# xytpai/kfunca

Measured on AMD Instinct MI355X. Metric: bf16 GEMM TFLOP/s + causal-attn fwd+bwd tokens/s, higher is better.
Workload: dtype bf16

## Files before the change

### kfunca_amd/csrc/device/attention.hip

```cpp
#include <math.h>
#include <stdlib.h>

#include <algorithm>
#include <type_traits>

#include "common.h"

namespace kf {

typedef __attribute__((ext_vector_type(8))) __bf16 bf16x8;
typedef __attribute__((ext_vector_type(8))) _Float16 f16x8;
typedef __attribute__((ext_vector_type(4))) short s16x4;
typedef __attribute__((ext_vector_type(8))) short s16x8;
typedef __attribute__((ext_vector_type(16))) float f32x16;
typedef __attribute__((ext_vector_type(4))) float f32x4;

struct AttnArgs {
    const char *q, *k, *v, *o, *d_o;
    char *out, *dq, *dk, *dv;
    float *lse;
    const float *lse_r;
    float *delta;
    float *nlse, *ndelta;
    int64_t B, H, Sq, Skv, D;
// ... 735 lines not shown
    char *slab = smem + DQ_RING * FTILE + wid * DQ_RING * DQ_SLAB;
    int vo[DB][2];
#pragma unroll
    for (int d = 0; d < DB; ++d) {
        vo[d][0] = a_tr_lane_off(d * 32, 0);
        vo[d][1] = a_tr_lane_off(d * 32, 1);
    }
    const int grp = lane >> 4, qq = (lane >> 2) & 3, pp = lane & 3, h = grp >> 1;
    const unsigned smem_u = (unsigned)(uintptr_t)(const __attribute__((address_space(3))) char *)smem;
    const int sp = grp & 1;
    const unsigned ds_rd = smem_u + (unsigned)(slab - smem) + sp * 1024 + 64 * ((2 * h + (qq >> 1)) ^ (2 * sp)) + 32 * (qq & 1) + 16 * (pp & 1) + 8 * (pp >> 1);
    int ds_src[2];
#pragma unroll
    for (int pc = 0; pc < 2; ++pc) ds_src[pc] = pc * 1024 + (((lane >> 2) ^ (2 * pc)) * 4 + (lane & 3)) * 16;
    const int krow = lane >> 4, kpos = lane & 15;
#pragma nounroll
  for (int pass = 0; pass < (a.persist ? 2 * a.persist : 1); ++pass) {
    const int xp = xb0 + (pass >> 1) * nwx;
    const int xb = ((pass & 1) != (a.persist_rev != 0)) ? nxb - 1 - xp : xp;
    const int qblk = nxb - 1 - xb;
    const int64_t q0 = (int64_t)qblk * FQ, qw = q0 + wid * 32;
    const bool active = qw < a.Sq;
    const int sl = (int)(qw >> 5);
    f32x16 dq[DB];
#pragma unroll
    for (int d = 0; d < DB; ++d)
#pragma unroll
        for (int e = 0; e < 16; ++e) dq[d][e] = 0.f;
    const int64_t q_end = q0 + FQ < a.Sq ? q0 + FQ : a.Sq;
    const int64_t kv_end = a.Skv < q_end ? a.Skv : q_end;
    const int nt = (int)((kv_end + ABK - 1) / ABK);
    const char *dsg = a.ds + ((bh - a.bh0) * a.ds_pair + ds_row_base(qblk, a.ds_nkb, a.ds_tri) + wid) * DS_TILE;
    const int kwb_last = (int)(a.ds_nkb * 8 - 1);
    const int slw = qblk * 8 + wid;
    auto stage = [&](int tile, int slot) {
        const int tl = tile < nt ? tile : nt - 1;
        const int kfirst = tl * ABK, klast = (int)a.Skv - 1 - kfirst;
        const char *kg = Kg + (int64_t)kfirst * a.lk.sr;
#pragma unroll
        for (int i = 0; i < 2; ++i) {
            const int row0 = (wid * 2 + i) * 4, row = row0 + krow;
            const int chunk = kpos ^ (((row & 3) << 2) | ((row >> 2) & 3));
            const int srow = row < klast ? row : klast;
            if (D == AD || chunk < D / 8)
                __builtin_amdgcn_global_load_lds((const __attribute__((address_space(1))) void *)(kg + (int64_t)srow * a.lk.sr + chunk * 16),
                                                 (__attribute__((address_space(3))) void *)(smem + slot * FTILE + row0 * AROW), 16, 0, 0);
        }
#pragma unroll
        for (int hf = 0; hf < 2; ++hf) {
            int kwb = 2 * tl + hf;
            kwb = kwb < kwb_last ? kwb : kwb_last;
            kwb = kwb <= slw ? kwb : (slw < kwb_last ? slw : kwb_last);
            const char *tg = dsg + (int64_t)kwb * 8 * DS_TILE;
#pragma unroll
            for (int pc = 0; pc < 2; ++pc)
                __builtin_amdgcn_global_load_lds((const __attribute__((address_space(1))) void *)(tg + ds_src[pc]),
                                                 (__attribute__((address_space(3))) void *)(slab + slot * DQ_SLAB + hf * DS_TILE + pc * 1024), 16, 0, 0);
        }
    };
    stage(0, 0);
    stage(1, 1);
    for (int t = 0; t < nt; ++t) {
        asm volatile("s_waitcnt vmcnt(6)" ::: "memory");
        __builtin_amdgcn_s_barrier();
        asm volatile("" ::: "memory");
        stage(t + 2, (t + 2) % DQ_RING);
        const char *kt = smem + (t % DQ_RING) * FTILE;
        const unsigned dsb = ds_rd + (unsigned)((t % DQ_RING) * DQ_SLAB);
        if (active && 2 * t <= sl && !KF_MUT(3, t == 0 && qblk == nxb - 1)) {
            dq_step<BF, 0, 0, DB>(kt, vo, dsb, dq);
            dq_step<BF, 0, 1, DB>(kt, vo, dsb, dq);
            if (2 * t + 1 <= sl) {
                dq_step<BF, 1, 0, DB>(kt, vo, dsb, dq);
                dq_step<BF, 1, 1, DB>(kt, vo, dsb, dq);
            }
        }
    }
    asm volatile("s_waitcnt vmcnt(0)" ::: "memory");
    __syncthreads();
    if (active) a_store_rows<BF, DB>(smem + wid * 32 * OPAD, a.dq + a_head(a.ldq, bh, a.H) + qw * a.ldq.sr, dq, a.scale, a.ldq.sr,
                                     (int)(a.Sq - qw < 32 ? a.Sq - qw : 32));
    if (a.persist) __syncthreads();
  }
}

constexpr int BQS = 32;

constexpr int K4B = 128;
constexpr int K4SL = 2 * BQS * AROW + 256;
constexpr int K4PAIR = 2 * K4SL;
constexpr int K4LDS = 4 * K4PAIR;
constexpr bool K4_SPREAD = true;
static_assert(K4LDS >= 4 * 32 * OPAD, "epilogue slabs must fit");

template <int OFF>
__device__ __forceinline__ void k4_rows4(unsigned e, unsigned o, s16x8 (&f)[4]) {
    asm volatile("ds_read_b128 %0, %4 offset:%c6\n\tds_read_b128 %1, %5 offset:%c6\n\t"
                 "ds_read_b128 %2, %4 offset:%c7\n\tds_read_b128 %3, %5 offset:%c7"
                 : "=&v"(f[0]), "=&v"(f[1]), "=&v"(f[2]), "=&v"(f[3])
                 : "v"(e), "v"(o), "n"(OFF), "n"(OFF + 512)
                 : "memory");
}
template <int OFF>
__device__ __forceinline__ void k4_rowc(unsigned lr, f32x4 (&c)[4]) {
    asm volatile("ds_read_b128 %0, %4 offset:%c5\n\tds_read_b128 %1, %4 offset:%c6\n\t"
                 "ds_read_b128 %2, %4 offset:%c7\n\tds_read_b128 %3, %4 offset:%c8"
                 : "=&a"(c[0]), "=&a"(c[1]), "=&a"(c[2]), "=&a"(c[3])
                 : "v"(lr), "n"(OFF), "n"(OFF + 32), "n"(OFF + 64), "n"(OFF + 96)
                 : "memory");
}
struct K4Tr { s16x4 lo[4], hi[4]; };
template <int OFF>
__device__ __forceinline__ void k4_tr4(unsigned t0, unsigned t1, K4Tr &t) {
    asm volatile("ds_read_b64_tr_b16 %0, %8 offset:%c10\n\tds_read_b64_tr_b16 %1, %9 offset:%c10\n\t"
                 "ds_read_b64_tr_b16 %2, %8 offset:%c11\n\tds_read_b64_tr_b16 %3, %9 offset:%c11\n\t"
                 "ds_read_b64_tr_b16 %4, %8 offset:%c12\n\tds_read_b64_tr_b16 %5, %9 offset:%c12\n\t"
                 "ds_read_b64_tr_b16 %6, %8 offset:%c13\n\tds_read_b64_tr_b16 %7, %9 offset:%c13"
                 : "=&v"(t.lo[0]), "=&v"(t.hi[0]), "=&v"(t.lo[1]), "=&v"(t.hi[1]), "=&v"(t.lo[2]), "=&v"(t.hi[2]), "=&v"(t.lo[3]), "=&v"(t.hi[3])
                 : "v"(t0), "v"(t1), "n"(OFF), "n"(OFF + 512), "n"(OFF + 1024), "n"(OFF + 1536)
                 : "memory");
}
template <int N>
__device__ __forceinline__ void k4_wait4(s16x8 (&f)[4]) {
    asm volatile("s_waitcnt lgkmcnt(%c4)" : "+v"(f[0]), "+v"(f[1]), "+v"(f[2]), "+v"(f[3]) : "n"(N) : "memory");
}
template <int N>
__device__ __forceinline__ void k4_wait4c(s16x8 (&f)[4], f32x4 (&c)[4]) {
    asm volatile("s_waitcnt lgkmcnt(%c8)"
                 : "+v"(f[0]), "+v"(f[1]), "+v"(f[2]), "+v"(f[3]), "+a"(c[0]), "+a"(c[1]), "+a"(c[2]), "+a"(c[3])
                 : "n"(N)
                 : "memory");
}
template <int N>
__device__ __forceinline__ void k4_wait_tr(K4Tr &a) {
    asm volatile("s_waitcnt lgkmcnt(%c8)"
                 : "+v"(a.lo[0]), "+v"(a.hi[0]), "+v"(a.lo[1]), "+v"(a.hi[1]), "+v"(a.lo[2]), "+v"(a.hi[2]), "+v"(a.lo[3]), "+v"(a.hi[3])
                 : "n"(N)
                 : "memory");
}
template <bool BF>
__device__ __forceinline__ typename AFrag<BF>::type k4_frag(const K4Tr &t, int d) {
    s16x8 r;
    r[0] = t.lo[d][0]; r[1] = t.lo[d][1]; r[2] = t.lo[d][2]; r[3] = t.lo[d][3];
    r[4] = t.hi[d][0]; r[5] = t.hi[d][1]; r[6] = t.hi[d][2]; r[7] = t.hi[d][3];
    return __builtin_bit_cast(typename AFrag<BF>::type, r);
}
__device__ __forceinline__ f32x16 k4_acc(const f32x4 (&c)[4]) {
    f32x16 r;
#pragma unroll
    for (int g = 0; g < 4; ++g)
#pragma unroll
        for (int j = 0; j < 4; ++j) r[4 * g + j] = c[g][j];
    return r;
}

template <int OFF>
__device__ __forceinline__ void k4_rows4a(unsigned e, unsigned o, s16x8 (&f)[4]) {
    asm volatile("ds_read_b128 %0, %4 offset:%c6\n\tds_read_b128 %1, %5 offset:%c6\n\t"
                 "ds_read_b128 %2, %4 offset:%c7\n\tds_read_b128 %3, %5 offset:%c7"
                 : "=&a"(f[0]), "=&a"(f[1]), "=&a"(f[2]), "=&a"(f[3])
                 : "v"(e), "v"(o), "n"(OFF), "n"(OFF + 512)
                 : "memory");
}
template <int OFF>
__device__ __forceinline__ void k4_rowcv(unsigned lr, f32x4 (&c)[4]) {
    asm volatile("ds_read_b128 %0, %4 offset:%c5\n\tds_read_b128 %1, %4 offset:%c6\n\t"
// ... 1408 lines not shown
        return with_flags([&](auto BF, auto SQ) { return launch(attn_fwd_w4_kernel<BF, SQ>, grid, 256, KF_FWD_W4_LDS_BYTES, st, a); }, bf, sq);
    }
    KF_REQUIRE(!lays, KF_ERR_UNSUPPORTED, "kf_attn_fwd_strided: this shape / stride combination has no matrix-core kernel (ragged lengths want K and V with one row stride)");
    if (f32_mfma) {
        const size_t ldsx = std::max((size_t)2 * XK * (D + 4), (size_t)4 * 32 * (D + 4)) * sizeof(float);
        const int64_t nxx = (Sq + XQ - 1) / XQ;
        a.persist = pair_flag(nxx);
        KF_PROF("attn_fwd_f32_mfma", st);
        return launch(D == 128 ? attn_fwd_f32_mfma_kernel<128> : attn_fwd_f32_mfma_kernel<64>, (unsigned)((a.persist ? nxx / 2 : nxx) * B * H), 256, ldsx, st, a);
    }
    const int DP = (int)D + 1;
    const size_t lds = sizeof(float) * ((size_t)GQ * DP + (size_t)GK * DP + (size_t)GK * D + (size_t)GQ * (GK + 1) + GQ);
    KF_PROF("attn_fwd_generic", st);
    return launch(dtype == KF_F32 ? attn_fwd_generic_kernel<float> : bf ? attn_fwd_generic_kernel<bf16_t> : attn_fwd_generic_kernel<f16_t>,
                  dim3((unsigned)((Sq + GQ - 1) / GQ), (unsigned)(B * H)), 256, lds, st, a);
}

extern "C" int kf_attn_fwd(int dtype, int64_t B, int64_t H, int64_t Sq, int64_t Skv, int64_t D, const void *q,
                           const void *k, const void *v, void *o, float *lse, void *stream) {
    return kf_attn_fwd_scaled(dtype, B, H, Sq, Skv, D, D > 0 ? 1.0f / sqrtf((float)D) : 1.0f, q, k, v, o, lse, stream);
}

extern "C" int kf_attn_fwd_scaled(int dtype, int64_t B, int64_t H, int64_t Sq, int64_t Skv, int64_t D, float scale, const void *q,
                                  const void *k, const void *v, void *o, float *lse, void *stream) {
    return attn_fwd_impl(dtype, B, H, H, Sq, Skv, D, scale, q, k, v, o, lse, nullptr, stream);
}

static int attn_fwd_strided_impl(int dtype, int64_t B, int64_t H, int64_t Hkv, int64_t Sq, int64_t Skv, int64_t D, float scale, const void *q,
                                 const kf_attn_layout *lq, const void *k, const kf_attn_layout *lk, const void *v, const kf_attn_layout *lv,
                                 void *o, const kf_attn_layout *lo, float *lse, void *stream) {
    KF_REQUIRE(mfma16_ok(dtype, Sq, Skv, D), KF_ERR_UNSUPPORTED,
               "kf_attn_fwd_strided: strided layouts are served by the 16-bit matrix-core kernels only (D = 64 or 128; Skv >= Sq, or Sq, Skv multiples of 128)");
    AttnArgs::Lay lays[4];
    KF_REQUIRE(lay_from(lq, 2, lays[0]) && lay_from(lk, 2, lays[1]) && lay_from(lv, 2, lays[2]) && lay_from(lo, 2, lays[3]), KF_ERR_INVALID,
               "kf_attn_fwd_strided: strides must be non-negative multiples of 8 elements");
    KF_REQUIRE(((uintptr_t)q | (uintptr_t)k | (uintptr_t)v | (uintptr_t)o) % 16 == 0, KF_ERR_INVALID, "kf_attn_fwd_strided: operands must be 16-byte aligned");
    return attn_fwd_impl(dtype, B, H, Hkv, Sq, Skv, D, scale, q, k, v, o, lse, lays, stream);
}

extern "C" int kf_attn_fwd_strided(int dtype, int64_t B, int64_t H, int64_t Sq, int64_t Skv, int64_t D, float scale, const void *q,
                                   const kf_attn_layout *lq, const void *k, const kf_attn_layout *lk, const void *v, const kf_attn_layout *lv,
                                   void *o, const kf_attn_layout *lo, float *lse, void *stream) {
    return attn_fwd_strided_impl(dtype, B, H, H, Sq, Skv, D, scale, q, lq, k, lk, v, lv, o, lo, lse, stream);
}

extern "C" int kf_attn_bwd_workspace_bytes(int dtype, int64_t B, int64_t H, int64_t Sq, int64_t Skv, int64_t D,
                                           size_t *bytes) {
    KF_REQUIRE(bytes, KF_ERR_INVALID, "kf_attn_bwd_workspace_bytes: null out pointer");
    int rc = check_common("kf_attn_bwd_workspace_bytes", dtype, B, H, Sq, Skv, D);
    if (rc != KF_OK) return rc;
    *bytes = bwd_stats_bytes(B * H, Sq);
    if (mfma16_ok(dtype, Sq, Skv, D) && B * H > 0) {
        const DsPlan ds = ds_plan(B * H, Sq, Skv, ds_cap());
        *bytes += ds_bytes(ds.group, Sq, Skv, ds.tri);
    }
    return KF_OK;
}

static size_t gqa_part_bytes(int dtype, int64_t B, int64_t H, int64_t Hkv, int64_t Skv, int64_t D) {
    return H == Hkv ? 0 : a_align((size_t)B * H * Skv * D * (dtype == KF_F32 ? 4 : 2));
}

static int attn_dkv_group_sum(int dtype, int64_t B, int64_t Hkv, int64_t Skv, int64_t D, int G, const char *pk, const char *pv, void *dk, void *dv,
                              AttnArgs::Lay ldk, AttnArgs::Lay ldv, hipStream_t st) {
    constexpr int R = 4;
    const int es = dtype == KF_F32 ? 4 : 2, vec = 16 / es;
    const bool wide = D % vec == 0 && (((uintptr_t)dk | (uintptr_t)dv) % 16 == 0) &&
                      ((ldk.sb | ldk.sh | ldk.sr | ldv.sb | ldv.sh | ldv.sr) % 16 == 0);
    const int nparts = (int)(wide ? D / vec : D);
    int lg = 0;
    while ((1 << lg) < nparts && lg < 6) ++lg;
    const int64_t nrows = B * Hkv * Skv, rows_per_block = (int64_t)(256 >> lg) * R;
    const unsigned grid = (unsigned)((nrows + rows_per_block - 1) / rows_per_block);
    KF_PROF("attn_bwd_dkv_group_sum", st);
    auto go = [&](auto t) {
        using T = decltype(t);
        return wide ? launch(attn_dkv_group_sum_kernel<T, 16 / sizeof(T), R>, grid, 256, 0, st, pk, pv, (char *)dk, (char *)dv, ldk, ldv, nrows, Skv, Hkv, G,
                             nparts, lg)
                    : launch(attn_dkv_group_sum_kernel<T, 1, R>, grid, 256, 0, st, pk, pv, (char *)dk, (char *)dv, ldk, ldv, nrows, Skv, Hkv, G, nparts, lg);
    };
    return dtype == KF_F32 ? go(float{}) : dtype == KF_BF16 ? go(bf16_t{}) : go(f16_t{});
}

static int attn_bwd_kernels(int dtype, int64_t B, int64_t H, int64_t Hkv, int64_t Sq, int64_t Skv, int64_t D, float scale, const void *q, const void *k,
                            const void *v, const void *o, const float *lse, const void *d_o, void *dq, void *dk, void *dv, const AttnArgs::Lay *lays,
                            void *workspace, size_t workspace_bytes, void *stream) {
    int rc = check_common("kf_attn_bwd", dtype, B, H, Sq, Skv, D);
    if (rc != KF_OK) return rc;
    if (B * H == 0 || Sq == 0 || Skv == 0) return KF_OK;
    KF_REQUIRE(q && k && v && o && lse && d_o && dq && dk && dv, KF_ERR_INVALID, "kf_attn_bwd: null operand");
    const size_t stats = bwd_stats_bytes(B * H, Sq), part = gqa_part_bytes(dtype, B, H, Hkv, Skv, D);
    const size_t need = stats + 2 * part;
    KF_REQUIRE(workspace && workspace_bytes >= need, KF_ERR_WORKSPACE, "kf_attn_bwd: workspace of at least %zu bytes required, got %zu", need, workspace_bytes);
    AttnArgs a;
    if ((rc = attn_args(a, B, H, Hkv, Sq, Skv, D, scale, lays, 8)) != KF_OK) return rc;
    a.q = (const char *)q; a.k = (const char *)k; a.v = (const char *)v; a.o = (const char *)o; a.d_o = (const char *)d_o;
    a.dq = (char *)dq; a.dk = (char *)dk; a.dv = (char *)dv;
    if (part) {
        a.dk = (char *)workspace + stats;
        a.dv = a.dk + part;
        a.ldk = a.ldv = lay_contig(H, Skv, D, 2);
    }
    a.lse_r = lse; a.delta = (float *)workspace;
    a.Sqc = stat_rows(Sq);
    a.nlse = (float *)((char *)workspace + a_align((size_t)B * H * Sq * sizeof(float)));
    a.ndelta = (float *)((char *)a.nlse + a_align((size_t)B * H * a.Sqc * sizeof(float)));
    hipStream_t st = as_stream(stream);
    const int64_t nbh = B * H, nrows = nbh * Sq;
    const bool bf = dtype == KF_BF16, d64 = D == 64;
    const bool tiled = mfma_ok(dtype, Sq, Skv, D);
    const bool dkv_w4 = ((tiled && Skv % K5B == 0) || w4_any_ok(dtype, Sq, Skv, D)) && a.lk.sr == a.lv.sr && a.ldk.sr == a.ldv.sr &&
                        (uint64_t)(Sq + 32) * (uint64_t)std::max(a.lq.sr, a.ldo.sr) < (1ull << 32) && (uint64_t)K5B * (uint64_t)std::max(a.lk.sr, a.ldk.sr) < (1ull << 31) &&
                        (uint64_t)((const char *)a.ndelta - (const char *)a.nlse) < (1ull << 31) && !knob(KNOB_ATTN_DKV_V4);
    const DsPlan ds = ds_plan(nbh, Sq, Skv, workspace_bytes - need);
    const bool keep_ds = ds.group > 0;
    const bool mfma16 = tiled || (dkv_w4 && keep_ds);
    const bool f32_mfma = dtype == KF_F32 && (D == 64 || D == 128) && Sq % 32 == 0 && Skv % 32 == 0;
    if (mfma16) {
        const bool dkv_sq = dkv_w4 && D == AD && knob(KNOB_ATTN_SCALED_OPERANDS);
        const float rscale = dkv_sq ? kLog2e : 1.0f / scale;
        {
            KF_PROF("attn_bwd_delta", st);
            const int64_t nrows_c = nbh * a.Sqc;
            rc = launch(bf ? attn_delta_kernel<true, 2> : attn_delta_kernel<false, 2>, (unsigned)((nrows_c + 31) / 32), 256, 0, st, a.o, a.d_o, a.delta,
                        nrows_c, a.lse_r, a.nlse, a.ndelta, rscale, a.lo, a.ldo, Sq, H, (int)(D / 8), a.Sqc);
            if (rc != KF_OK) return rc;
        }
        a.ds = keep_ds ? (char *)workspace + need : nullptr;
        a.ds_tri = ds.tri;
        a.ds_pair = ds_pair_tiles(Sq, Skv, ds.tri);
        a.ds_nkb = (Skv + 255) / 256;
        const int64_t nkb4 = Skv / K4B, nkb5 = (Skv + K5B - 1) / K5B, nxq = (Sq + FQ - 1) / FQ;
        const int64_t grp = keep_ds ? ds.group : nbh;
        for (int64_t bh0 = 0; bh0 < nbh; bh0 += grp) {
            a.bh0 = bh0;
            a.nbh = (int)std::min<int64_t>(grp, nbh - bh0);
            a.xcd_map = (a.nbh % 8 == 0) && !knob(KNOB_ATTN_NO_XCD);
            {
                a.persist_rev = 1;
                KF_PROF(d64 ? "attn_bwd_dkv_mfma_d64" : "attn_bwd_dkv_mfma", st);
                if (dkv_w4) {
                    a.persist = pair_flag(nkb5);
                    const dim3 grid((unsigned)((a.persist ? nkb5 / 2 : nkb5) * a.nbh));
                    a.nvwg = grid.x;
                    if (d64)
                        rc = with_flags([&](auto BF, auto DS) { return launch(attn_bwd_dkv_w4_kernel<BF, DS, false, true>, grid, 256, KF_DKV_W4_LDS_BYTES, st, a); },
                                        bf, keep_ds);
                    else
                        rc = with_flags([&](auto BF, auto DS, auto SQ) { return launch(attn_bwd_dkv_w4_kernel<BF, DS, SQ>, grid, 256, KF_DKV_W4_LDS_BYTES, st, a); },
                                        bf, keep_ds, dkv_sq);
                } else {
                    a.persist = pair_flag(nkb4);
                    const dim3 grid((unsigned)((a.persist ? nkb4 / 2 : nkb4) * a.nbh));
                    rc = with_flags([&](auto BF, auto DS, auto D64) { return launch(attn_bwd_dkv_v4_kernel<BF, DS, D64 ? 64 : 128>, grid, 256, K4LDS, st, a); },
                                    bf, keep_ds, d64);
                }
                if (rc != KF_OK) return rc;
            }
            a.persist = pair_flag(nxq);
            a.persist_rev = 0;
            const dim3 grid((unsigned)((a.persist ? nxq / 2 : nxq) * a.nbh));
            if (keep_ds) {
                KF_PROF(d64 ? "attn_bwd_dq_mfma_d64" : "attn_bwd_dq_mfma", st);
                rc = with_flags([&](auto BF, auto D64) { return launch(attn_bwd_dq_ds_kernel<BF, D64 ? 64 : 128>, grid, FNT, DQ_LDS, st, a); }, bf, d64);
            } else {
                KF_PROF(d64 ? "attn_bwd_dq_mfma_split_d64" : "attn_bwd_dq_mfma_split", st);
                rc = with_flags([&](auto BF, auto D64) { return launch(attn_bwd_dq_v2_kernel<BF, D64 ? 64 : 128>, grid, FNT, QLDS, st, a); }, bf, d64);
            }
            if (rc != KF_OK) return rc;
        }
        return KF_OK;
    }
    KF_REQUIRE(!lays, KF_ERR_UNSUPPORTED, "kf_attn_bwd_strided: this shape / stride / workspace combination has no matrix-core kernel (ragged lengths want room for dS)");
    const unsigned gd = (unsigned)((nrows + 3) / 4);
    if (f32_mfma) {
        {
            KF_PROF("attn_bwd_delta", st);
            rc = launch(attn_delta_generic_kernel<float>, gd, 256, 0, st, (const float *)o, (const float *)d_o, a.delta, nrows, (int)D);
            if (rc != KF_OK) return rc;
        }
        const size_t tiles = (size_t)2 * XK * (D + 4) * sizeof(float) + 256, slabs = (size_t)4 * 32 * (D + 4) * sizeof(float);
        const size_t ldsx = std::max(tiles, slabs);
        const int64_t nxq = (Sq + XQ - 1) / XQ, nkb = (Skv + XQ - 1) / XQ;
        {
            a.persist = pair_flag(nkb);
            KF_PROF("attn_bwd_dkv_f32_mfma", st);
            rc = launch(D == 128 ? attn_bwd_dkv_f32_mfma_kernel<128> : attn_bwd_dkv_f32_mfma_kernel<64>, (unsigned)((a.persist ? nkb / 2 : nkb) * B * H), 256, ldsx, st, a);
            if (rc != KF_OK) return rc;
        }
        a.persist = pair_flag(nxq);
        KF_PROF("attn_bwd_dq_f32_mfma", st);
        return launch(D == 128 ? attn_bwd_dq_f32_mfma_kernel<128> : attn_bwd_dq_f32_mfma_kernel<64>, (unsigned)((a.persist ? nxq / 2 : nxq) * B * H), 256, ldsx, st, a);
    }
    const int DP = (int)D + 1;
    const size_t lds = sizeof(float) * ((size_t)2 * GQ * DP + (size_t)2 * GK * DP + (size_t)2 * GQ * (GK + 1) + 2 * GK);
    const dim3 gq((unsigned)((Sq + GQ - 1) / GQ), (unsigned)(B * H)), gk((unsigned)((Skv + GQ - 1) / GQ), (unsigned)(B * H));
    KF_PROF("attn_bwd_generic", st);
    auto generic = [&](auto t) {
        using T = decltype(t);
        int r = launch(attn_delta_generic_kernel<T>, gd, 256, 0, st, (const T *)o, (const T *)d_o, a.delta, nrows, (int)D);
        if (r == KF_OK) r = launch(attn_bwd_generic_kernel<T, 0>, gq, 256, lds, st, a);
        if (r == KF_OK) r = launch(attn_bwd_generic_kernel<T, 1>, gk, 256, lds, st, a);
        return r;
    };
    return dtype == KF_F32 ? generic(float{}) : bf ? generic(bf16_t{}) : generic(f16_t{});
}

static int attn_bwd_impl(int dtype, int64_t B, int64_t H, int64_t Hkv, int64_t Sq, int64_t Skv, int64_t D, float scale, const void *q, const void *k,
                         const void *v, const void *o, const float *lse, const void *d_o, void *dq, void *dk, void *dv, const AttnArgs::Lay *lays,
                         void *workspace, size_t workspace_bytes, void *stream) {
    const int rc = attn_bwd_kernels(dtype, B, H, Hkv, Sq, Skv, D, scale, q, k, v, o, lse, d_o, dq, dk, dv, lays, workspace, workspace_bytes, stream);
    if (rc != KF_OK || Hkv == H || B * H == 0 || Sq == 0 || Skv == 0) return rc;
    const int es = dtype == KF_F32 ? 4 : 2;
    const size_t part = gqa_part_bytes(dtype, B, H, Hkv, Skv, D);
    const char *pk = (const char *)workspace + bwd_stats_bytes(B * H, Sq), *pv = pk + part;
    return attn_dkv_group_sum(dtype, B, Hkv, Skv, D, (int)(H / Hkv), pk, pv, dk, dv, lays ? lays[6] : lay_contig(Hkv, Skv, D, es),
                              lays ? lays[7] : lay_contig(Hkv, Skv, D, es), as_stream(stream));
}

extern "C" int kf_attn_bwd(int dtype, int64_t B, int64_t H, int64_t Sq, int64_t Skv, int64_t D, const void *q,
                           const void *k, const void *v, const void *o, const float *lse, const void *d_o, void *dq,
                           void *dk, void *dv, void *workspace, size_t workspace_bytes, void *stream) {
    return kf_attn_bwd_scaled(dtype, B, H, Sq, Skv, D, D > 0 ? 1.0f / sqrtf((float)D) : 1.0f, q, k, v, o, lse, d_o, dq, dk, dv, workspace,
                              workspace_bytes, stream);
}

extern "C" int kf_attn_bwd_scaled(int dtype, int64_t B, int64_t H, int64_t Sq, int64_t Skv, int64_t D, float scale, const void *q,
                                  const void *k, const void *v, const void *o, const float *lse, const void *d_o, void *dq,
                                  void *dk, void *dv, void *workspace, size_t workspace_bytes, void *stream) {
    return attn_bwd_impl(dtype, B, H, H, Sq, Skv, D, scale, q, k, v, o, lse, d_o, dq, dk, dv, nullptr, workspace, workspace_bytes, stream);
}

static int attn_bwd_strided_impl(int dtype, int64_t B, int64_t H, int64_t Hkv, int64_t Sq, int64_t Skv, int64_t D, float scale, const void *q,
                                 const kf_attn_layout *lq, const void *k, const kf_attn_layout *lk, const void *v, const kf_attn_layout *lv,
                                 const void *o, const kf_attn_layout *lo, const float *lse, const void *d_o, const kf_attn_layout *ldo, void *dq,
                                 const kf_attn_layout *ldq, void *dk, const kf_attn_layout *ldk, void *dv, const kf_attn_layout *ldv,
                                 void *workspace, size_t workspace_bytes, void *stream) {
    KF_REQUIRE(mfma16_ok(dtype, Sq, Skv, D), KF_ERR_UNSUPPORTED,
               "kf_attn_bwd_strided: strided layouts are served by the 16-bit matrix-core kernels only (D = 64 or 128; Skv >= Sq, or Sq, Skv multiples of 128)");
    AttnArgs::Lay lays[8];
    const kf_attn_layout *in[8] = {lq, lk, lv, lo, ldo, ldq, ldk, ldv};
    for (int i = 0; i < 8; ++i)
        KF_REQUIRE(lay_from(in[i], 2, lays[i]), KF_ERR_INVALID, "kf_attn_bwd_strided: strides must be non-negative multiples of 8 elements");
    KF_REQUIRE(((uintptr_t)q | (uintptr_t)k | (uintptr_t)v | (uintptr_t)o | (uintptr_t)d_o | (uintptr_t)dq | (uintptr_t)dk | (uintptr_t)dv) % 16 == 0,
               KF_ERR_INVALID, "kf_attn_bwd_strided: operands must be 16-byte aligned");
    return attn_bwd_impl(dtype, B, H, Hkv, Sq, Skv, D, scale, q, k, v, o, lse, d_o, dq, dk, dv, lays, workspace, workspace_bytes, stream);
}
// ... 78 lines not shown
```

### kfunca_amd/csrc/device/common.h

```cpp
#pragma once

#include <hip/hip_runtime.h>
#include <stdint.h>
#include <stdio.h>
#include <string.h>

#include <type_traits>

#include "kfunca_hip.h"

namespace kf {

void set_error(const char *fmt, ...);

#define KF_HIP_TRY(expr)                                                                              \
    do {                                                                                              \
        hipError_t e_ = (expr);                                                                       \
        if (e_ != hipSuccess) {                                                                       \
            ::kf::set_error("%s failed: %s (%s:%d)", #expr, hipGetErrorString(e_), __FILE__, __LINE__); \
            (void)hipGetLastError();  \
            return KF_ERR_HIP;                                                                        \
        }                                                                                             \
    } while (0)

#define KF_REQUIRE(cond, code, ...)        \
    do {                                   \
        if (!(cond)) {                     \
            ::kf::set_error(__VA_ARGS__);  \
            return (code);                 \
        }                                  \
    } while (0)

#define KF_LAUNCH_CHECK()                                                                    \
    do {                                                                                     \
        hipError_t e_ = hipGetLastError();                                                   \
        if (e_ != hipSuccess) {                                                              \
            ::kf::set_error("kernel launch failed: %s (%s:%d)", hipGetErrorString(e_), __FILE__, __LINE__); \
            return KF_ERR_HIP;                                                               \
        }                                                                                    \
    } while (0)

static inline int dtype_size(int dt) {
    switch (dt) {
    case KF_BOOL: case KF_U8: case KF_I8: return 1;
    case KF_I16: case KF_F16: case KF_BF16: return 2;
    case KF_I32: case KF_F32: return 4;
    case KF_I64: case KF_F64: return 8;
    default: return 0;
    }
}

struct alignas(2) bf16_t { uint16_t x; };
struct alignas(2) f16_t { uint16_t x; };

__device__ __forceinline__ float bf16_to_f32(bf16_t v) { return __uint_as_float(((uint32_t)v.x) << 16); }
__device__ __forceinline__ bf16_t f32_to_bf16(float f) {
    bf16_t r;
    uint32_t u = __float_as_uint(f);
    if ((u & 0x7fffffffu) > 0x7f800000u) { r.x = 0x7FC0; return r; }
    r.x = (uint16_t)((u + 0x7FFFu + ((u >> 16) & 1u)) >> 16);
    return r;
}
__device__ __forceinline__ uint32_t f32x2_to_bf16x2_hw(float lo, float hi) {
    uint32_t r;
    asm("v_cvt_pk_bf16_f32 %0, %1, %2" : "=v"(r) : "v"(lo), "v"(hi));
    return r;
}
__device__ __forceinline__ float f16_to_f32(f16_t v) {
    _Float16 h;
    __builtin_memcpy(&h, &v.x, 2);
    return (float)h;
}
__device__ __forceinline__ f16_t f32_to_f16(float f) {
    _Float16 h = (_Float16)f;
    f16_t r;
    __builtin_memcpy(&r.x, &h, 2);
    return r;
}

constexpr int kWave = 64;

struct ProfScope {
    const char *name;
    hipStream_t st;
    void *rec;
    ProfScope(const char *name, hipStream_t st);
    ~ProfScope();
};
#define KF_PROF(name, st) ::kf::ProfScope kf_prof_scope_((name), (st))

static inline hipStream_t as_stream(void *s) { return reinterpret_cast<hipStream_t>(s); }

enum Knob {
    KNOB_ATTN_NO_XCD, KNOB_ATTN_NO_DEFER, KNOB_ATTN_NO_PAIR, KNOB_ATTN_SPLIT_BWD, KNOB_GEMM_NO_SPLITK, KNOB_GEMM_NO_GROUP,
    KNOB_ATTN_DS_CAP_MB, KNOB_ATTN_FWD_V3, KNOB_ATTN_DKV_V4, KNOB_ATTN_SCALED_OPERANDS, KNOB_GEMM_NO_PAD, KNOB_EW_ALIGNED_ONLY, KNOB_ATTN_DS_TRI, KNOB_COUNT
};
bool knob(Knob k);
long knob_int(Knob k, long dflt);

int ensure_dynamic_lds(const void *kernel, int bytes);

template <typename... P, typename... A>
static inline int launch(void (*kernel)(P...), dim3 grid, dim3 block, size_t lds, hipStream_t st, A &&...args) {
    if (lds > 0) {
        const int rc = ensure_dynamic_lds((const void *)kernel, (int)lds);
        if (rc != KF_OK) return rc;
    }
    kernel<<<grid, block, lds, st>>>(static_cast<A &&>(args)...);
    KF_LAUNCH_CHECK();
    return KF_OK;
}

template <typename F> static inline int with_flags(F &&f) { return f(); }
template <typename F, typename... B> static inline int with_flags(F &&f, bool b, B... rest) {
    return b ? with_flags([&](auto... x) { return f(std::true_type{}, x...); }, rest...)
             : with_flags([&](auto... x) { return f(std::false_type{}, x...); }, rest...);
}

int sort_with_key_bits(int dtype, const void *keys_in, void *keys_out, int64_t *pos_out, int64_t nseg, int64_t n, int descending, void *workspace,
                       size_t workspace_bytes, void *stream, int key_bits);

}
```

### kfunca_amd/csrc/device/runtime.hip

```cpp
#include <stdarg.h>

#include "common.h"

namespace kf {
static thread_local char g_err[1024] = "";
void set_error(const char *fmt, ...) {
    va_list ap;
    va_start(ap, fmt);
    vsnprintf(g_err, sizeof(g_err), fmt, ap);
    va_end(ap);
}
}

#include <algorithm>
#include <mutex>
#include <string>
#include <vector>
namespace kf {
struct ProfRec { std::string name; hipEvent_t e0, e1; };
static bool g_prof_on = false;
static int g_capturing = 0;
static std::mutex g_prof_mu;
static std::vector<ProfRec *> g_prof_recs;
ProfScope::ProfScope(const char *n, hipStream_t s) : name(n), st(s), rec(nullptr) {
    if (!g_prof_on || g_capturing) return;
    ProfRec *r = new ProfRec();
    r->name = n;
    if (hipEventCreate(&r->e0) != hipSuccess || hipEventCreate(&r->e1) != hipSuccess) { delete r; return; }
    hipEventRecord(r->e0, s);
    rec = r;
}
ProfScope::~ProfScope() {
    if (!rec) return;
    ProfRec *r = (ProfRec *)rec;
    hipEventRecord(r->e1, st);
    std::lock_guard<std::mutex> lk(g_prof_mu);
    g_prof_recs.push_back(r);
}
struct ProfSum { std::string name; double ms; int64_t n; std::vector<float> each; };
static std::vector<ProfSum> g_prof_sums;
static void prof_collect() {
    std::lock_guard<std::mutex> lk(g_prof_mu);
    for (ProfRec *r : g_prof_recs) {
        float ms = 0.f;
        hipEventSynchronize(r->e1);
        hipEventElapsedTime(&ms, r->e0, r->e1);
        hipEventDestroy(r->e0);
        hipEventDestroy(r->e1);
        bool found = false;
        for (auto &s : g_prof_sums)
            if (s.name == r->name) { s.ms += ms; s.n += 1; if (s.each.size() < 65536) s.each.push_back(ms); found = true; break; }
        if (!found) g_prof_sums.push_back({r->name, (double)ms, 1, {ms}});
        delete r;
    }
    g_prof_recs.clear();
}
}

#include <stdlib.h>
namespace kf {
static const char *const g_knob_names[KNOB_COUNT] = {
    "KF_ATTN_NO_XCD", "KF_ATTN_NO_DEFER", "KF_ATTN_NO_PAIR", "KF_ATTN_SPLIT_BWD", "KF_GEMM_NO_SPLITK", "KF_GEMM_NO_GROUP",
    "KF_ATTN_DS_CAP_MB", "KF_ATTN_FWD_V3", "KF_ATTN_DKV_V4", "KF_ATTN_SCALED_OPERANDS", "KF_GEMM_NO_PAD", "KF_EW_ALIGNED_ONLY", "KF_ATTN_DS_TRI"};
static std::mutex g_knob_mu;
static bool g_knob_loaded = false;
static bool g_knob_set[KNOB_COUNT];
static long g_knob_val[KNOB_COUNT];
static void knobs_load_locked() {
    for (int i = 0; i < KNOB_COUNT; ++i) {
        const char *e = getenv(g_knob_names[i]);
        g_knob_set[i] = e != nullptr;
        g_knob_val[i] = e ? strtol(e, nullptr, 10) : 0;
    }
    g_knob_loaded = true;
}
bool knob(Knob k) {
    if (!g_knob_loaded) {
        std::lock_guard<std::mutex> lk(g_knob_mu);
        if (!g_knob_loaded) knobs_load_locked();
    }
    return g_knob_set[k];
}
long knob_int(Knob k, long dflt) { return knob(k) ? g_knob_val[k] : dflt; }

struct LdsAttr { const void *fn; int dev; int bytes; };
static std::mutex g_lds_mu;
static std::vector<LdsAttr> g_lds_attrs;
int ensure_dynamic_lds(const void *kernel, int bytes) {
    int dev = 0;
    KF_HIP_TRY(hipGetDevice(&dev));
    std::lock_guard<std::mutex> lk(g_lds_mu);
    for (auto &a : g_lds_attrs)
        if (a.fn == kernel && a.dev == dev) {
            if (a.bytes >= bytes) return KF_OK;
            KF_HIP_TRY(hipFuncSetAttribute(kernel, hipFuncAttributeMaxDynamicSharedMemorySize, bytes));
            a.bytes = bytes;
            return KF_OK;
        }
    KF_HIP_TRY(hipFuncSetAttribute(kernel, hipFuncAttributeMaxDynamicSharedMemorySize, bytes));
    g_lds_attrs.push_back({kernel, dev, bytes});
    return KF_OK;
}
}

using namespace kf;

extern "C" {

int kf_knobs_reload(void) {
    std::lock_guard<std::mutex> lk(g_knob_mu);
    knobs_load_locked();
    return KF_OK;
}

int kf_profile_enable(int on) {
    KF_REQUIRE(!(on && g_capturing), KF_ERR_INVALID, "kf_profile_enable: a stream capture is open (timing events would be recorded into the graph)");
    g_prof_on = on != 0;
    return KF_OK;
}
int kf_profile_reset(void) {
    prof_collect();
    std::lock_guard<std::mutex> lk(g_prof_mu);
    g_prof_sums.clear();
    return KF_OK;
}
int kf_profile_count(int *n) {
    KF_REQUIRE(n, KF_ERR_INVALID, "kf_profile_count: null out pointer");
    prof_collect();
    *n = (int)g_prof_sums.size();
    return KF_OK;
}
int kf_profile_get(int i, char name[64], double *total_ms, int64_t *launches) {
    KF_REQUIRE(name && total_ms && launches, KF_ERR_INVALID, "kf_profile_get: null out pointer");
    prof_collect();
    KF_REQUIRE(i >= 0 && i < (int)g_prof_sums.size(), KF_ERR_INVALID, "kf_profile_get: index %d out of range", i);
    snprintf(name, 64, "%s", g_prof_sums[i].name.c_str());
    *total_ms = g_prof_sums[i].ms;
    *launches = g_prof_sums[i].n;
    return KF_OK;
}

int kf_profile_samples(int i, float *ms, int capacity, int *written) {
    KF_REQUIRE(ms && written && capacity >= 0, KF_ERR_INVALID, "kf_profile_samples: null out pointer");
    prof_collect();
    KF_REQUIRE(i >= 0 && i < (int)g_prof_sums.size(), KF_ERR_INVALID, "kf_profile_samples: index %d out of range", i);
    const int n = std::min<int>(capacity, (int)g_prof_sums[i].each.size());
// ... 198 lines not shown
```

Measured before the change: 7.707 million.

## Add persistent dQ kernel that prefetches next pass tiles across work items

Adds a persistent attention-backward dQ kernel launched with about one workgroup per CU. It keeps a single K/dS staging ring that carries prefetches across pass and work-item boundaries, so loads for the next block overlap the tail and epilogue of the current one. dQ is written through a swizzled LDS slab as coalesced 64-bit stores. This aims to remove the pipeline drain/refill and launch tail of one workgroup per q-block, at the cost of more complex synchronisation and a grid-size choice that depends on the CU count.

```diff
diff --git a/kfunca_amd/csrc/device/attention.hip b/kfunca_amd/csrc/device/attention.hip
--- a/kfunca_amd/csrc/device/attention.hip
+++ b/kfunca_amd/csrc/device/attention.hip
@@ -841,6 +841,178 @@
                                      (int)(a.Sq - qw < 32 ? a.Sq - qw : 32));
     if (a.persist) __syncthreads();
   }
+}
+
+struct DqPass {
+    const char *Kg;
+    const char *dsg;
+    char *dq;
+    int nt, qblk;
+};
+
+typedef __attribute__((ext_vector_type(2))) unsigned u32x2;
+template <bool BF, int DB>
+__device__ __forceinline__ void dq_store_rows(unsigned slab, char *dst, const f32x16 (&acc)[DB], float mul, int64_t rs, int nrows) {
+    static_assert(DB % 2 == 0, "two column blocks per round");
+    const int lane = threadIdx.x & 63, xl = lane & 31, hl = lane >> 5;
+#pragma unroll
+    for (int half = 0; half < DB / 2; ++half) {
+#pragma unroll
+        for (int dd = 0; dd < 2; ++dd)
+#pragma unroll
+            for (int gq = 0; gq < 4; ++gq) {
+                const f32x16 &x = acc[2 * half + dd];
+                const uint32_t h0 = a_cvt16<BF>(x[4 * gq + 0] * mul), h1 = a_cvt16<BF>(x[4 * gq + 1] * mul);
+                const uint32_t h2 = a_cvt16<BF>(x[4 * gq + 2] * mul), h3 = a_cvt16<BF>(x[4 * gq + 3] * mul);
+                u32x2 w;
+                w.x = h0 | (h1 << 16);
+                w.y = h2 | (h3 << 16);
+                const int unit = dd * 8 + 2 * gq + hl;
+                asm volatile("ds_write_b64 %0, %1" : : "v"(slab + (unsigned)(xl * 128 + ((unit ^ (xl & 15)) << 3))), "v"(w) : "memory");
+            }
+        u32x2 w[8];
+#pragma unroll
+        for (int i = 0; i < 8; ++i) {
+            const int id = lane + 64 * i, row = id >> 4, unit = id & 15;
+            asm volatile("ds_read_b64 %0, %1" : "=v"(w[i]) : "v"(slab + (unsigned)(row * 128 + ((unit ^ (row & 15)) << 3))) : "memory");
+        }
+        asm volatile("s_waitcnt lgkmcnt(0)" : "+v"(w[0]), "+v"(w[1]), "+v"(w[2]), "+v"(w[3]), "+v"(w[4]), "+v"(w[5]), "+v"(w[6]), "+v"(w[7]) : : "memory");
+#pragma unroll
+        for (int i = 0; i < 8; ++i) {
+            const int id = lane + 64 * i, row = id >> 4, unit = id & 15;
+            if (row < nrows) *(uint2 *)(dst + (int64_t)row * rs + half * 128 + unit * 8) = make_uint2(w[i].x, w[i].y);
+        }
+    }
+}
+
+template <bool BF, int D>
+__global__ __launch_bounds__(FNT, 2) void attn_bwd_dq_ds_carry_kernel(const AttnArgs a) {
+    constexpr int DB = D / 32;
+    extern __shared__ __attribute__((aligned(16))) char smem[];
+    const int lane = threadIdx.x & 63, wid = __builtin_amdgcn_readfirstlane(threadIdx.x >> 6);
+    const int nxb = (int)((a.Sq + FQ - 1) / FQ);
+    const int nwx = a.persist ? nxb / (2 * a.persist) : nxb;
+    const int npass = a.persist ? 2 * a.persist : 1;
+    const unsigned nvwg = (unsigned)nwx * (unsigned)a.nbh;
+    char *slab = smem + DQ_RING * FTILE + wid * DQ_RING * DQ_SLAB;
+    int vo[DB][2];
+#pragma unroll
+    for (int d = 0; d < DB; ++d) {
+        vo[d][0] = a_tr_lane_off(d * 32, 0);
+        vo[d][1] = a_tr_lane_off(d * 32, 1);
+    }
+    const int grp = lane >> 4, qq = (lane >> 2) & 3, pp = lane & 3, h = grp >> 1;
+    const unsigned smem_u = (unsigned)(uintptr_t)(const __attribute__((address_space(3))) char *)smem;
+    const int sp = grp & 1;
+    const unsigned ds_rd = smem_u + (unsigned)(slab - smem) + sp * 1024 + 64 * ((2 * h + (qq >> 1)) ^ (2 * sp)) + 32 * (qq & 1) + 16 * (pp & 1) + 8 * (pp >> 1);
+    int ds_src[2];
+#pragma unroll
+    for (int pc = 0; pc < 2; ++pc) ds_src[pc] = pc * 1024 + (((lane >> 2) ^ (2 * pc)) * 4 + (lane & 3)) * 16;
+    const int krow = lane >> 4, kpos = lane & 15;
+    const int kwb_last = (int)(a.ds_nkb * 8 - 1);
+    auto pass_of = [&](unsigned vwg, int pass, DqPass &p) {
+        int xb0;
+        int64_t bhl;
+        a_block_map(nwx, a.nbh, a.xcd_map, xb0, bhl, vwg);
+        const unsigned bh = (unsigned)(bhl + a.bh0), b = bh / (unsigned)a.H, hd = bh - b * (unsigned)a.H;
+        const int xp = xb0 + (pass >> 1) * nwx;
+        const int xb = ((pass & 1) != (a.persist_rev != 0)) ? nxb - 1 - xp : xp;
+        p.qblk = nxb - 1 - xb;
+        const int64_t q0 = (int64_t)p.qblk * FQ;
+        const int64_t q_end = q0 + FQ < a.Sq ? q0 + FQ : a.Sq;
+        const int64_t kv_end = a.Skv < q_end ? a.Skv : q_end;
+        p.nt = (int)((kv_end + ABK - 1) / ABK);
+        p.Kg = a.k + (int64_t)b * a.lk.sb + (int64_t)(hd / (unsigned)a.G) * a.lk.sh;
+        p.dq = a.dq + (int64_t)b * a.ldq.sb + (int64_t)hd * a.ldq.sh;
+        p.dsg = a.ds + ((bhl * a.ds_pair) + ds_row_base(p.qblk, a.ds_nkb, a.ds_tri) + wid) * DS_TILE;
+    };
+    auto stage = [&](const DqPass &p, int tl, int slot) {
+        const int kfirst = tl * ABK, klast = (int)a.Skv - 1 - kfirst;
+        const char *kg = p.Kg + (int64_t)kfirst * a.lk.sr;
+        const int slw = p.qblk * 8 + wid;
+#pragma unroll
+        for (int i = 0; i < 2; ++i) {
+            const int row0 = (wid * 2 + i) * 4, row = row0 + krow;
+            const int chunk = kpos ^ (((row & 3) << 2) | ((row >> 2) & 3));
+            const int srow = row < klast ? row : klast;
+            if (D == AD || chunk < D / 8)
+                __builtin_amdgcn_global_load_lds((const __attribute__((address_space(1))) void *)(kg + (int64_t)srow * a.lk.sr + chunk * 16),
+                                                 (__attribute__((address_space(3))) void *)(smem + slot * FTILE + row0 * AROW), 16, 0, 0);
+        }
+#pragma unroll
+        for (int hf = 0; hf < 2; ++hf) {
+            int kwb = 2 * tl + hf;
+            kwb = kwb < kwb_last ? kwb : kwb_last;
+            kwb = kwb <= slw ? kwb : (slw < kwb_last ? slw : kwb_last);
+            const char *tg = p.dsg + (int64_t)kwb * 8 * DS_TILE;
+#pragma unroll
+            for (int pc = 0; pc < 2; ++pc)
+                __builtin_amdgcn_global_load_lds((const __attribute__((address_space(1))) void *)(tg + ds_src[pc]),
+                                                 (__attribute__((address_space(3))) void *)(slab + slot * DQ_SLAB + hf * DS_TILE + pc * 1024), 16, 0, 0);
+        }
+    };
+    DqPass fp;
+    unsigned fv = blockIdx.x;
+    int fpass = 0, ft = 0, ahead = 0;
+    bool live = fv < nvwg;
+    if (live) pass_of(fv, 0, fp);
+    auto fetch = [&](int slot) {
+        if (!live) return;
+        stage(fp, ft, slot);
+        ++ahead;
+        if (++ft < fp.nt) return;
+        ft = 0;
+        if (++fpass == npass) {
+            fpass = 0;
+            fv += gridDim.x;
+        }
+        live = fv < nvwg;
+        if (live) pass_of(fv, fpass, fp);
+    };
+    fetch(0);
+    fetch(1);
+    int s = 0;
+#pragma nounroll
+    for (unsigned vwg = blockIdx.x; vwg < nvwg; vwg += gridDim.x) {
+#pragma nounroll
+        for (int pass = 0; pass < npass; ++pass) {
+            DqPass cp;
+            pass_of(vwg, pass, cp);
+            const int64_t qw = (int64_t)cp.qblk * FQ + wid * 32;
+            const bool active = qw < a.Sq;
+            const int sl = (int)(qw >> 5);
+            f32x16 dq[DB];
+#pragma unroll
+            for (int d = 0; d < DB; ++d)
+#pragma unroll
+                for (int e = 0; e < 16; ++e) dq[d][e] = 0.f;
+            for (int t = 0; t < cp.nt; ++t) {
+                if (ahead >= 2)
+                    asm volatile("s_waitcnt vmcnt(6)" ::: "memory");
+                else
+                    asm volatile("s_waitcnt vmcnt(0)" ::: "memory");
+                __builtin_amdgcn_s_barrier();
+                asm volatile("" ::: "memory");
+                fetch(s == 0 ? DQ_RING - 1 : s - 1);
+                const char *kt = smem + s * FTILE;
+                const unsigned dsb = ds_rd + (unsigned)(s * DQ_SLAB);
+                if (active && 2 * t <= sl && !KF_MUT(3, t == 0 && cp.qblk == nxb - 1)) {
+                    dq_step<BF, 0, 0, DB>(kt, vo, dsb, dq);
+                    dq_step<BF, 0, 1, DB>(kt, vo, dsb, dq);
+                    if (2 * t + 1 <= sl) {
+                        dq_step<BF, 1, 0, DB>(kt, vo, dsb, dq);
+                        dq_step<BF, 1, 1, DB>(kt, vo, dsb, dq);
+                    }
+                }
+                --ahead;
+                s = s == DQ_RING - 1 ? 0 : s + 1;
+            }
+            if (active)
+                dq_store_rows<BF, DB>(smem_u + (unsigned)(slab - smem) + (unsigned)((s == 0 ? DQ_RING - 1 : s - 1) * DQ_SLAB), cp.dq + qw * a.ldq.sr, dq, a.scale, a.ldq.sr,
+                                      (int)(a.Sq - qw < 32 ? a.Sq - qw : 32));
+        }
+    }
+    asm volatile("s_waitcnt vmcnt(0)" ::: "memory");
 }
 
 constexpr int BQS = 32;
@@ -2415,7 +2587,16 @@
     return dtype == KF_F32 ? go(float{}) : dtype == KF_BF16 ? go(bf16_t{}) : go(f16_t{});
 }
 
-static int attn_bwd_kernels(int dtype, int64_t B, int64_t H, int64_t Hkv, int64_t Sq, int64_t Skv, int64_t D, float scale, const void *q, const void *k,
+static long device_cus() {
+    static int cus = 0;
+    if (cus == 0) {
+        int dev = 0, n = 0;
+        cus = hipGetDevice(&dev) == hipSuccess && hipDeviceGetAttribute(&n, hipDeviceAttributeMultiprocessorCount, dev) == hipSuccess && n > 0 ? n : 256;
+    }
+    return cus;
+}
+
+static int attn_bwd_kernels(int dtype,int64_t B, int64_t H, int64_t Hkv, int64_t Sq, int64_t Skv, int64_t D, float scale, const void *q, const void *k,
                             const void *v, const void *o, const float *lse, const void *d_o, void *dq, void *dk, void *dv, const AttnArgs::Lay *lays,
                             void *workspace, size_t workspace_bytes, void *stream) {
     int rc = check_common("kf_attn_bwd", dtype, B, H, Sq, Skv, D);
@@ -2495,7 +2676,14 @@
             const dim3 grid((unsigned)((a.persist ? nxq / 2 : nxq) * a.nbh));
             if (keep_ds) {
                 KF_PROF(d64 ? "attn_bwd_dq_mfma_d64" : "attn_bwd_dq_mfma", st);
-                rc = with_flags([&](auto BF, auto D64) { return launch(attn_bwd_dq_ds_kernel<BF, D64 ? 64 : 128>, grid, FNT, DQ_LDS, st, a); }, bf, d64);
+                if (knob(KNOB_ATTN_DQ_NO_CARRY)) {
+                    rc = with_flags([&](auto BF, auto D64) { return launch(attn_bwd_dq_ds_kernel<BF, D64 ? 64 : 128>, grid, FNT, DQ_LDS, st, a); }, bf, d64);
+                } else {
+                    unsigned real = (unsigned)std::min<long>(grid.x, std::max<long>(1, knob_int(KNOB_ATTN_GRID_WGS, device_cus())));
+                    if (a.xcd_map) real = std::max(8u, real - real % 8);
+                    rc = with_flags([&](auto BF, auto D64) { return launch(attn_bwd_dq_ds_carry_kernel<BF, D64 ? 64 : 128>, real, FNT, DQ_LDS, st, a); },
+                                    bf, d64);
+                }
             } else {
                 KF_PROF(d64 ? "attn_bwd_dq_mfma_split_d64" : "attn_bwd_dq_mfma_split", st);
                 rc = with_flags([&](auto BF, auto D64) { return launch(attn_bwd_dq_v2_kernel<BF, D64 ? 64 : 128>, grid, FNT, QLDS, st, a); }, bf, d64);
diff --git a/kfunca_amd/csrc/device/common.h b/kfunca_amd/csrc/device/common.h
--- a/kfunca_amd/csrc/device/common.h
+++ b/kfunca_amd/csrc/device/common.h
@@ -93,7 +93,10 @@
 
 enum Knob {
     KNOB_ATTN_NO_XCD, KNOB_ATTN_NO_DEFER, KNOB_ATTN_NO_PAIR, KNOB_ATTN_SPLIT_BWD, KNOB_GEMM_NO_SPLITK, KNOB_GEMM_NO_GROUP,
-    KNOB_ATTN_DS_CAP_MB, KNOB_ATTN_FWD_V3, KNOB_ATTN_DKV_V4, KNOB_ATTN_SCALED_OPERANDS, KNOB_GEMM_NO_PAD, KNOB_EW_ALIGNED_ONLY, KNOB_ATTN_DS_TRI, KNOB_COUNT
+    KNOB_ATTN_DS_CAP_MB, KNOB_ATTN_FWD_V3, KNOB_ATTN_DKV_V4, KNOB_ATTN_SCALED_OPERANDS, KNOB_GEMM_NO_PAD, KNOB_EW_ALIGNED_ONLY, KNOB_ATTN_DS_TRI,
+    KNOB_ATTN_DQ_NO_CARRY,
+    KNOB_ATTN_GRID_WGS,
+    KNOB_COUNT
 };
 bool knob(Knob k);
 long knob_int(Knob k, long dflt);
diff --git a/kfunca_amd/csrc/device/runtime.hip b/kfunca_amd/csrc/device/runtime.hip
--- a/kfunca_amd/csrc/device/runtime.hip
+++ b/kfunca_amd/csrc/device/runtime.hip
@@ -61,7 +61,8 @@
 namespace kf {
 static const char *const g_knob_names[KNOB_COUNT] = {
     "KF_ATTN_NO_XCD", "KF_ATTN_NO_DEFER", "KF_ATTN_NO_PAIR", "KF_ATTN_SPLIT_BWD", "KF_GEMM_NO_SPLITK", "KF_GEMM_NO_GROUP",
-    "KF_ATTN_DS_CAP_MB", "KF_ATTN_FWD_V3", "KF_ATTN_DKV_V4", "KF_ATTN_SCALED_OPERANDS", "KF_GEMM_NO_PAD", "KF_EW_ALIGNED_ONLY", "KF_ATTN_DS_TRI"};
+    "KF_ATTN_DS_CAP_MB", "KF_ATTN_FWD_V3", "KF_ATTN_DKV_V4", "KF_ATTN_SCALED_OPERANDS", "KF_GEMM_NO_PAD", "KF_EW_ALIGNED_ONLY", "KF_ATTN_DS_TRI",
+    "KF_ATTN_DQ_NO_CARRY", "KF_ATTN_GRID_WGS"};
 static std::mutex g_knob_mu;
 static bool g_knob_loaded = false;
 static bool g_knob_set[KNOB_COUNT];
```

New measurement: 7.736 million, median of 5. About the same (+0.4%).
